# thowell/CALIPSO.jl

Hardware: AMD Instinct MI355X
Metric: Newton steps/sec (n~5k KKT) (higher is better)
Workload: dtype f64; 1 GPU; C3 synthetic dense conic QP: nx=2500 ne=1500 nc=1000 (400 R+ + 200 x SOC3), n=5000 condensed, N=8500 unreduced; ONE system per GPU stepped sequentially (replicas at N > 1); 1 LDL^T factorisation, 6 refinement round(s) per step; refinement_rounds=6

## Files before the change

calipso.jl_amd/csrc/api.hip:

```cpp
#include <algorithm>
#include <array>
#include <atomic>
#include <cmath>
#include <mutex>
#include <cstdio>
#include <cstdlib>
#include <cstring>

#include "internal.hpp"
#include "device_utils.hpp"
#include "host_logic.hpp"

using namespace calipso;

namespace calipso {
int check(H* s, hipError_t e, const char* what) {
    char buf[512];
    snprintf(buf, sizeof buf, "%s: %s", what, hipGetErrorString(e));
    if (s) s->err = buf;
    return CALIPSO_ERR_HIP;
}
bool lds_attribute(const void* kernel, int bytes) {
    static std::mutex mu;
    static std::map<std::pair<const void*, int>, std::pair<int, int>> done;
// ... 107 lines not shown
            const int st = d.ne + s->h_soc_start[j], dim = s->h_soc_dim[j];
            int lo = d.nx, hi = 0;
            for (int k = st; k < st + dim; ++k) if (zr[2 * (size_t)k + 1] > zr[2 * (size_t)k]) { lo = std::min(lo, zr[2 * (size_t)k]); hi = std::max(hi, zr[2 * (size_t)k + 1]); }
            for (int k = st; k < st + dim; ++k) { zr[2 * (size_t)k] = hi > lo ? lo : 0; zr[2 * (size_t)k + 1] = hi > lo ? hi : 0; }
        }
        if (spec->n_blocks < 1 || spec->block_start[0] != 1) { s->err = "calipso_hip_create_structured: hessian_block_start must begin with 1"; return CALIPSO_ERR_ARGUMENT; }
        for (int64_t b = 0; b < spec->n_blocks; ++b) {
            const int64_t c0 = spec->block_start[b], c1 = b + 1 < spec->n_blocks ? spec->block_start[b + 1] : nx + 1;
            if (c1 <= c0 || c1 > nx + 1) { s->err = "calipso_hip_create_structured: hessian_block_start must be increasing within 1..nx"; return CALIPSO_ERR_ARGUMENT; }
            for (int64_t c = c0; c < c1; ++c) lr[(size_t)c - 1] = (int)c1 - 2;
        }
        s->h_zrow = zr; s->h_lreach = lr;
        std::vector<int>& reach = s->h_reach;
        reach = lr;
        std::vector<int> ext((size_t)d.nx, -1);
        for (int k = 0; k < d.m; ++k) if (zr[2 * (size_t)k + 1] > zr[2 * (size_t)k]) ext[(size_t)zr[2 * (size_t)k]] = std::max(ext[(size_t)zr[2 * (size_t)k]], zr[2 * (size_t)k + 1] - 1);
        int run = -1;
        for (int j = 0; j < d.nx; ++j) { run = std::max(run, ext[(size_t)j]); if (run >= j) reach[(size_t)j] = std::max(reach[(size_t)j], run); }
        if (!calipso::blocks_plan(d, zr, lr, plan, s->err)) return CALIPSO_ERR_ARGUMENT;
        s->compact = true;
        s->blocks_zero_cell = plan.spacked - 1;
    }
    const bool cp = s->compact;
    std::vector<std::pair<double**, size_t>> carve;
    auto SL = [&](double** pp, size_t count) { carve.push_back({pp, count ? count : 1}); };
    double* icount_d = nullptr;
    SL(&s->Lxx, cp ? 1 : NX * NX); SL(&s->Lsym, cp ? plan.packed : NX * NX); SL(&s->Z, cp ? 1 : M * NX);
    SL(&s->fx, NX); SL(&s->gyx, NX); SL(&s->hzx, NX); SL(&s->gh, M);
    SL(&s->cone_product, NC); SL(&s->cone_target, NC); SL(&s->barrier_gradient, NC);
    SL(&s->dscal, 64); SL(&s->refpart, std::max((NE + NC + 255) / 256 + 1, M + 2) + (size_t)d.n_wide);
    SL(&s->solution, N); SL(&s->candidate, N); SL(&s->lambda, NE); SL(&s->parameters, (size_t)d.np);
    SL(&s->residual, N); SL(&s->residual_error, N); SL(&s->step, N); SL(&s->step_correction, N);
    SL(&s->saved_point, N); SL(&s->saved_g, NE); SL(&s->saved_h, NC);
    SL(&s->residual_symmetric, n); SL(&s->step_symmetric, n); SL(&s->merit_gradient, n);
    SL(&s->S, cp ? plan.spacked : NPd * NPd); SL(&s->Dx, NPd); SL(&s->Ypanel, cp ? 1 : NPd * NB);
    SL(&s->Tinv, cp ? 1 : calipso::tinv_doubles(d.NP)); SL(&s->Ttmp, cp ? 1 : NPd * 1024); SL(&s->zf2, NPd); SL(&s->WH, cp ? 1 : NC * NX);
    SL(&s->Wfac, (cp || !calipso::wform_layout_ok(d.NP, calipso::trsv_block(d.NP, 512))) ? 1 : NPd * NPd / 2);
    SL(&s->wz, NC); SL(&s->kzz, NC);
    SL(&s->Wsoc, (size_t)woff); SL(&s->Bsoc, (size_t)woff); SL(&s->socwork, (size_t)2 * woff);
    SL(&icount_d, 32);
    double* krange_d = nullptr;
    const size_t KG = (NX + 15) / 16;
    SL(&krange_d, 2 * KG);
    double* zrow_d = nullptr;
    SL(&zrow_d, M);
    const size_t maxdim = std::max(std::max(NX, M), NPd);
    SL(&s->gemv_partial, cp ? 1 : std::max(64 * maxdim, ((NX + 15) / 16) * M + ((M + 1023) / 1024) * NX));
    SL(&s->vtmp, 4 * std::max(N, NPd));
    SL(&s->xbuf, NPd); SL(&s->zf, NPd); SL(&s->t1, M); SL(&s->t2, M);
    SL(&s->zsx, M); SL(&s->w1, NX); SL(&s->w2, NX); SL(&s->lxv, NX);
    SL(&s->lgp, NX * d.np); SL(&s->gp, NE * d.np); SL(&s->hp, NC * d.np);
    SL(&s->jacobian_parameters, N * d.np); SL(&s->solution_sensitivity, N * d.np);
    SL(&s->qp.q, NX); SL(&s->qp.bh, M);
    size_t total = 0;
    for (auto& c : carve) total += (c.second + 31) & ~(size_t)31;
    CK(hipMalloc((void**)&s->slab, total * sizeof(double)));
    CK(hipMemsetAsync(s->slab, 0, total * sizeof(double), s->stream));
    s->slab_doubles = total;
    {
        size_t off = 0;
        for (auto& c : carve) { *c.first = s->slab + off; off += (c.second + 31) & ~(size_t)31; }
    }
    s->icount = reinterpret_cast<int*>(icount_d);
    s->krange = reinterpret_cast<int*>(krange_d);
    s->zrow = reinterpret_cast<int*>(zrow_d);
    s->gx = s->Z; s->hx = s->Z + NE; s->g = s->gh; s->hc = s->gh + NE;
    s->Lf = s->S;
    schur_plan(s);
    rc |= dalloc(s, &s->cone.soc_start, (size_t)d.n_soc); rc |= dalloc(s, &s->cone.soc_dim, (size_t)d.n_soc);
    rc |= dalloc(s, &s->cone.soc_woff, (size_t)d.n_soc); rc |= dalloc(s, &s->cone.entry_soc, NC);
    rc |= dalloc(s, &s->cone.wide, (size_t)d.n_wide);
    std::vector<int> zgrp;
    calipso::solve_tail_plan(d, s->h_soc_start, s->h_soc_dim, zgrp);
    if (zgrp.size() >= 2) { rc |= dalloc(s, &s->zgrp, zgrp.size()); s->n_zgrp = (int)zgrp.size() - 1; }
    rc |= dalloc(s, &s->gate, (size_t)4);
    if (rc) return CALIPSO_ERR_HIP;
    CK(hipHostMalloc((void**)&s->hscal, 64 * sizeof(double), hipHostMallocMapped | hipHostMallocCoherent));
    CK(hipHostMalloc((void**)&s->hicount, 64 * sizeof(int), hipHostMallocMapped | hipHostMallocCoherent));
    CK(hipHostMalloc((void**)&s->hseq, 64, hipHostMallocMapped | hipHostMallocCoherent));
    CK(hipHostGetDevicePointer((void**)&s->hscal_dev, s->hscal, 0));
    CK(hipHostGetDevicePointer((void**)&s->hicount_dev, s->hicount, 0));
    CK(hipHostGetDevicePointer((void**)&s->hseq_dev, s->hseq, 0));
    s->hseq[0] = 0;
    CK(hipStreamSynchronize(s->stream));
    {
        std::vector<int> kr(4 * KG);
        for (size_t g = 0; g < KG; ++g) { kr[4 * g] = 0; kr[4 * g + 1] = d.ne; kr[4 * g + 2] = 0; kr[4 * g + 3] = d.nc; }
        CK(hipMemcpy(s->krange, kr.data(), sizeof(int) * kr.size(), hipMemcpyHostToDevice));
    }
    if (s->zgrp) CK(hipMemcpy(s->zgrp, zgrp.data(), sizeof(int) * zgrp.size(), hipMemcpyHostToDevice));
    if (d.n_soc) {
        CK(hipMemcpy(s->cone.soc_start, s->h_soc_start.data(), sizeof(int) * d.n_soc, hipMemcpyHostToDevice));
        CK(hipMemcpy(s->cone.soc_dim, s->h_soc_dim.data(), sizeof(int) * d.n_soc, hipMemcpyHostToDevice));
        CK(hipMemcpy(s->cone.soc_woff, s->h_soc_woff.data(), sizeof(int) * d.n_soc, hipMemcpyHostToDevice));
    }
    if (d.n_wide) {
        std::vector<int> wide;
        for (int j = 0; j < d.n_soc; ++j) if (s->h_soc_dim[j] > 4) wide.push_back(j);
        CK(hipMemcpy(s->cone.wide, wide.data(), sizeof(int) * wide.size(), hipMemcpyHostToDevice));
    }
    std::vector<int> es((size_t)std::max(1, d.nc), -1);
    for (int j = 0; j < d.n_soc; ++j)
        for (int k = 0; k < s->h_soc_dim[j]; ++k) es[s->h_soc_start[j] + k] = j;
    if (d.nc) CK(hipMemcpy(s->cone.entry_soc, es.data(), sizeof(int) * d.nc, hipMemcpyHostToDevice));
    s->hpoint.assign(N, 0.0);
    s->hparams.assign((size_t)d.np, 0.0);
    Options& o = s->opt;
#define OD(f) s->optd["opt." #f] = &o.f
    OD(residual_norm); OD(constraint_norm); OD(scaling_line_search); OD(iterative_refinement_tolerance); OD(central_path_initial);
    OD(central_path_update_tolerance); OD(central_path_scaling); OD(central_path_exponent); OD(penalty_initial); OD(penalty_scaling);
    OD(dual_initial); OD(residual_tolerance); OD(optimality_tolerance); OD(slack_tolerance); OD(equality_tolerance);
    OD(complementarity_tolerance); OD(min_regularization); OD(primal_regularization_initial); OD(dual_regularization_initial);
    OD(max_regularization); OD(dual_regularization); OD(dual_regularization_exponent); OD(scaling_regularization_initial);
    OD(scaling_regularization); OD(scaling_regularization_last); OD(min_central_path); OD(max_penalty); OD(constraint_tensor);
    OD(update_factorization); OD(violation_tolerance); OD(violation_exponent); OD(merit_tolerance); OD(merit_exponent);
    OD(armijo_tolerance); OD(machine_tolerance); OD(max_filter); OD(differentiate); OD(warmstart);
#undef OD
    const int mf = (int)o.max_filter;
    s->filter_theta.assign(mf, 1.0e8); s->filter_merit.assign(mf, 1.0e8);
    s->cache_theta.assign(mf, 1.0e8); s->cache_merit.assign(mf, 1.0e8);
    if (cp) {
        CK(hipStreamSynchronize(s->stream));
        int brc = calipso::blocks_install(s, plan);
        if (brc < 0) return brc;
        brc = calipso_hip_set_stage_parallel(s, 1, 1, nullptr);
        if (brc < 0) return brc;
// ... 1210 lines not shown
```

calipso.jl_amd/csrc/gemv.hip:

```cpp
#include "internal.hpp"
#include "device_utils.hpp"

namespace calipso {

struct BlockRanges { int b0, b1, b2, b3; };
__device__ __forceinline__ BlockRanges column_blocks(const Sparsity& sp, int col, int rows) {
    BlockRanges r = {0, (rows + 63) / 64, 0, 0};
    if (sp.kind == SP_DENSE) return r;
    if (sp.kind == SP_LXX) { r.b0 = max(0, col - sp.hb) / 64; r.b1 = (min(rows, col + sp.hb + 1) + 63) / 64; return r; }
    const int* k = sp.kr + 4 * (col / 16);
    const int elo = k[0], ehi = k[1], clo = k[2], chi = k[3];
    if (sp.kind == SP_GX) { r.b0 = elo / 64; r.b1 = ehi > elo ? (ehi + 63) / 64 : r.b0; return r; }
    if (sp.kind == SP_HX) { r.b0 = clo / 64; r.b1 = chi > clo ? (chi + 63) / 64 : r.b0; return r; }
    r.b0 = elo / 64; r.b1 = ehi > elo ? (ehi + 63) / 64 : r.b0;
    r.b2 = (sp.ne + clo) / 64; r.b3 = chi > clo ? (sp.ne + chi + 63) / 64 : r.b2;
    return r;
}
__device__ __forceinline__ bool block_active(const BlockRanges& r, int b) { return (b >= r.b0 && b < r.b1) || (b >= r.b2 && b < r.b3); }

template <int NV>
__device__ __forceinline__ void structured_column(const BlockRanges& br, int rows, int lane, const double* __restrict__ a, const double* const (&x)[NV],
                                                  double (&acc0)[NV], double (&acc1)[NV]) {
#pragma unroll
    for (int pass = 0; pass < 2; ++pass) {
// ... 254 lines not shown
    for (int q = 0; q < BOTH_RQ; ++q) if (block_active(br, r0 / 64 + q)) active |= 1u << q;
    for (int j = c0; j < c1; ++j) {
        const double* a = A + (size_t)j * ld;
        double z[BOTH_RQ];
#pragma unroll
        for (int q = 0; q < BOTH_RQ; ++q) { const int i = r0 + lane + 64 * q; z[q] = (i < rows && ((active >> q) & 1u)) ? a[i] : 0.0; }
        const double xj = x[j];
        double t0 = 0.0, t1 = 0.0;
#pragma unroll
        for (int q = 0; q < BOTH_RQ; q += 2) {
            t0 += z[q] * uu[q]; t1 += z[q + 1] * uu[q + 1];
            acc[q] += z[q] * xj; acc[q + 1] += z[q + 1] * xj;
        }
        const double t = wave_sum(t0 + t1);
        if (lane == 0) part_t[(size_t)blockIdx.y * cols + j] = t;
    }
#pragma unroll
    for (int q = 0; q < BOTH_RQ; ++q) { const int i = r0 + lane + 64 * q; if (i < rows) part_n[(size_t)cg * rows + i] = acc[q]; }
}

void gemv_both(calipso_hip_solver* s, int rows, int cols, const double* A, int ld, const double* x, const double* u, double* yn, double* yt, double beta_t, int kind) {
    if (rows == 0 || cols == 0) return;
    if (s->compact) { s->err = "internal: a dense mat-vec was requested on a structured handle"; s->ldl_failed = true; return; }
    const BatchSc B = batch_of(s);
    const int cw = BOTH_CW;
    const int ncg = (cols + cw - 1) / cw, nrr = (rows + 64 * BOTH_RQ - 1) / (64 * BOTH_RQ);
    double* part_n = s->gemv_partial;
    double* part_t = s->gemv_partial + (size_t)ncg * rows;
    hipLaunchKernelGGL(k_gemv_both, dim3((ncg + 3) / 4, nrr, B.b.n), dim3(256), 0, s->stream, B.b, sparsity_of(s, kind), rows, cols, cw, A, ld, x, u, part_n, part_t);
    hipLaunchKernelGGL(k_gemv_n_reduce, dim3((rows + 63) / 64, 1, B.b.n), dim3(256), 0, s->stream, B.b, rows, ncg, part_n, yn, 1.0, 0.0);
    hipLaunchKernelGGL(k_gemv_n_reduce, dim3((cols + 63) / 64, 1, B.b.n), dim3(256), 0, s->stream, B.b, cols, nrr, part_t, yt, 1.0, beta_t);
}

static void gemv_n_chunks(int rows, int cols, int& rb, int& nchunk, int& chunk) {
    rb = (rows + GN_ROWS - 1) / GN_ROWS;
    nchunk = (768 + rb - 1) / rb;
    if (nchunk > GN_MAXCHUNK) nchunk = GN_MAXCHUNK;
    if (nchunk > (cols + 15) / 16) nchunk = (cols + 15) / 16;
    if (nchunk < 1) nchunk = 1;
    chunk = (cols + nchunk - 1) / nchunk;
    nchunk = (cols + chunk - 1) / chunk;
    if (cols == 0) nchunk = 0;
}

int gemv_refine_pair(calipso_hip_solver* s, const double* x1, const double* x2, double* y1, double* y2, const double* xl, double* yl, bool defer_reduce) {
    const Dims& d = s->d;
    if (d.m == 0 || s->blocks.on || s->compact) {
        if (d.m) gemv_t2(s, d.m, d.nx, s->Z, d.m, x1, x2, y1, y2, SP_Z);
        gemv_n(s, d.nx, d.nx, s->Lxx, d.nx, xl, yl, 1.0, 0.0, SP_LXX);
        return 0;
    }
    int rb, nchunk, chunk;
    gemv_n_chunks(d.nx, d.nx, rb, nchunk, chunk);
    const int nt2 = (d.nx + 3) / 4;
    const BatchSc B = batch_of(s);
    const bool timed = s->time_matvec && !s->cur;
    if (timed) (void)hipEventRecord(s->ev[5], s->stream);
    const size_t xbytes = 2 * sizeof(double) * (size_t)d.m;
    const int lds_x = gemv_lds_x(xbytes);
    hipLaunchKernelGGL(k_gemv_t2_and_n, dim3(nt2 + rb * nchunk, 1, B.b.n), dim3(256), lds_x ? xbytes : 0, s->stream, B.b, sparsity_of(s, SP_Z), d.m, d.nx, s->Z, d.m, x1, x2, y1, y2, nt2,
                       sparsity_of(s, SP_LXX), rb, d.nx, d.nx, chunk, s->Lxx, d.nx, xl, s->gemv_partial, s->gate_epoch ? s->gate : (const int*)nullptr, s->gate_epoch, lds_x);
    if (timed) { (void)hipEventRecord(s->ev[6], s->stream); s->time_matvec = false; s->matvec_timed = true; }
    if (defer_reduce) return nchunk;
    hipLaunchKernelGGL(k_gemv_n_reduce, dim3((d.nx + 63) / 64, 1, B.b.n), dim3(256), 0, s->stream, B.b, d.nx, nchunk, s->gemv_partial, yl, 1.0, 0.0);
    return 0;
}

void gemv_n(calipso_hip_solver* s, int rows, int cols, const double* A, int ld, const double* x, double* y, double alpha, double beta, int kind, const double* add) {
    if (rows == 0) return;
    if (blocks_gemv_n(s, kind, x, y, alpha, beta)) { if (add) launch_add(s, y, add, rows); return; }
    if (s->compact) { s->err = "internal: a dense mat-vec was requested on a structured handle"; s->ldl_failed = true; return; }
    int rb, nchunk, chunk;
    gemv_n_chunks(rows, cols, rb, nchunk, chunk);
    const BatchSc B = batch_of(s);
    if (nchunk > 0)
        hipLaunchKernelGGL(k_gemv_n_partial, dim3(rb, nchunk, B.b.n), dim3(GN_ROWS), 0, s->stream, B.b, sparsity_of(s, kind), kind == SP_HX ? s->d.ne : 0, rows, cols, chunk, A, ld,
                           x, s->gemv_partial);
    hipLaunchKernelGGL(k_gemv_n_reduce, dim3((rows + 63) / 64, 1, B.b.n), dim3(256), 0, s->stream, B.b, rows, nchunk, s->gemv_partial, y, alpha, beta, add);
}

}
```

calipso.jl_amd/csrc/internal.hpp:

```cpp
#pragma once
#include <hip/hip_runtime.h>
#include <stdint.h>

#include <map>
#include <string>
#include <vector>

#include "../../include/calipso_hip.h"
#include "../../include/calipso_options.hpp"

namespace calipso {

constexpr int TILE = 128;
constexpr int NB = 64;
constexpr int MAX_SOC_DIM = 1024;
constexpr int TRSV_BLOCK = 2048;
inline int trsv_block(int NP, int limit = TRSV_BLOCK) {
    if (NP <= 512) return NP;
    int tb = 512;
    while (2 * tb <= limit && 2 * tb <= NP) tb *= 2;
    for (;; tb /= 2) { const int rem = NP % tb; if (tb == 512 || (rem & (rem - 1)) == 0) return tb; }
}
inline size_t tinv_doubles(int NP) {
    size_t most = 0;
// ... 96 lines not shown
    calipso::Options opt;
    calipso::Scalars sc;
    calipso::ConeDev cone;
    calipso::QpEval qp;
    calipso::Stats stats;
    struct calipso_hip_group* owner = nullptr;
    const calipso::BatchSc* cur = nullptr;
    double* slab = nullptr; size_t slab_doubles = 0;
    int device = 0;
    hipStream_t stream = nullptr;
    std::string err;
    calipso_callback_fn cb_inner = nullptr, cb_outer = nullptr;
    void* cb_user = nullptr;
    calipso_device_eval_fn dev_eval = nullptr;
    void* dev_eval_user = nullptr;
    calipso_device_block_eval_fn dev_block_eval = nullptr;
    void* dev_block_eval_user = nullptr;
    size_t scratch_bytes = 0;
    bool rhs_ahead = false, rhs_joined = false;
    double *evalL = nullptr, *evalZ = nullptr;
    std::map<std::string, double*> optd;
    std::vector<int> h_soc_start, h_soc_dim, h_soc_woff;
    std::vector<int64_t> h_nonneg, h_soc_ptr, h_soc_idx;
    double* Lxx = nullptr;
    double* Z = nullptr;
    double *gx = nullptr, *hx = nullptr;
    double* Lsym = nullptr;
    bool hessian_dirty = true;
    double *fx = nullptr, *gyx = nullptr, *hzx = nullptr;
    double* gh = nullptr;
    double *g = nullptr, *hc = nullptr;
    double *cone_product = nullptr, *cone_target = nullptr, *barrier_gradient = nullptr;
    double* dscal = nullptr;
    double* hscal = nullptr;
    double* hscal_dev = nullptr;
    unsigned long long* hseq = nullptr;
    unsigned long long* hseq_dev = nullptr;
    unsigned long long pub_seq = 0;
    double *jacobian_parameters = nullptr, *solution_sensitivity = nullptr;
    double *solution = nullptr, *candidate = nullptr, *lambda = nullptr, *parameters = nullptr;
    double *residual = nullptr, *residual_error = nullptr, *step = nullptr, *step_correction = nullptr, *saved_point = nullptr;
    double *residual_symmetric = nullptr, *step_symmetric = nullptr, *merit_gradient = nullptr;
    bool pad_done = false;
    double* Kdense = nullptr;
    double* S = nullptr;
    double* Dx = nullptr;
    double* refpart = nullptr;
    int refparts = 0;
    int* zgrp = nullptr; int n_zgrp = 0;
    int* gate = nullptr; int gate_epoch = 0; int gate_counter = 0;
    bool refine_defer = false, refine_pending = false;
    bool spec_ahead_ok = false;
    bool refine_local_done = false;
    double* Ypanel = nullptr;
    double* Tinv = nullptr;
    double* Ttmp = nullptr;
    double* zf2 = nullptr;
    double* Wfac = nullptr;
    double* WH = nullptr;
    double* wz = nullptr;
    double* kzz = nullptr;
    double* Wsoc = nullptr;
    double* Bsoc = nullptr;
    double* socwork = nullptr;
    int schur_nj = 8;
    int half_bandwidth = 0, band64 = 0;
    std::vector<int> h_reach;
    std::vector<int> h_zrow, h_lreach;
    calipso::StageBlocks blocks;
    bool blocks_effective = true;
    size_t blocks_zero_cell = 0;
    bool compact = false;
    calipso_hip_sparse* spS = nullptr;
    long long* spS_src = nullptr;
    bool spS_values_current = false;
    int* spS_inv = nullptr;
    int* d_reach = nullptr;
    bool stage_parallel = false;
    calipso::i64 structure_resets = 0;
    int* krange = nullptr;
    int* zrow = nullptr;
    int* icount = nullptr;
    int* hicount = nullptr;
    int* hicount_dev = nullptr;
    double* gemv_partial = nullptr;
    double* vtmp = nullptr;
    double *xbuf = nullptr, *zf = nullptr, *t1 = nullptr, *t2 = nullptr;
    double *zsx = nullptr;
    double *w1 = nullptr, *w2 = nullptr, *lxv = nullptr;
    double *saved_g = nullptr, *saved_h = nullptr;
    double *lgp = nullptr, *gp = nullptr, *hp = nullptr;
    std::vector<double> hparams;
    double* multi_rhs = nullptr;
    double* dsym_multi = nullptr;
    void* scatter_aux = nullptr;
    void* ldl_aux = nullptr;
    void* lfac_aux = nullptr;
    bool lfac_last = false;
    bool lfac_failed = false;
    double* Lf = nullptr;
    double* Hdense = nullptr; int* lu_ipiv = nullptr;
    hipEvent_t ev[16];
    hipStream_t stream2 = nullptr;
    bool ldl_publish = false;
    unsigned long long ldl_pub_seq = 0;
    bool factor_times_pending = false;
// ... 158 lines not shown
```

calipso.jl_amd/csrc/vectors.hip:

```cpp
#include <algorithm>
#include <mutex>

#include "internal.hpp"
#include "device_utils.hpp"

namespace calipso {

constexpr int RT = 1024;

__global__ void k_residual(BatchSc bt, Dims d, const double* __restrict__ w, const double* __restrict__ lam,
                           const double* __restrict__ fx, const double* __restrict__ gyx, const double* __restrict__ hzx,
                           const double* __restrict__ g, const double* __restrict__ hc, const double* __restrict__ prod,
                           const double* __restrict__ targ, double* __restrict__ res) {
    inst_shift(bt.b, w, lam, fx, gyx, hzx, g, hc, prod, targ, res);
    const Scalars sc = bt.scal(blockIdx.z);
    const int i = blockIdx.x * blockDim.x + threadIdx.x;
    if (i >= d.N) return;
    double v;
    if (i < d.orr()) {
        v = fx[i];
        v += gyx[i];
        v += hzx[i];
    } else if (i < d.os()) {
        const int k = i - d.orr();
// ... 982 lines not shown
    double m = 0.0;
    double qs[MD], qt[MD], qz[MD];
#pragma unroll
    for (int a = 0; a < MD; ++a) { qs[a] = 0.0; qt[a] = 0.0; qz[a] = 0.0; }
#pragma unroll
    for (int a = 0; a < MD; ++a) if (a < dim) {
        const int k = st + a;
        const double hs = (0.0 + sc.ep) * lvs[a] - lvz[a] - lvt[a];
        qs[a] = res_s[a] - hs;
        const double hz = zk[a] + (-lvs[a] + (0.0 - sc.ed) * lvz[a]);
        qz[a] = res_z[a] - hz;
        double ht;
        if (a == 0) {
            ht = t[0] * lvs[0] + (sl[0] - sc.ed) * lvt[0];
#pragma unroll
            for (int q = 1; q < MD; ++q) if (q < dim) ht += t[q] * lvs[q] + sl[q] * lvt[q];
        } else {
            ht = t[a] * lvs[0] + sl[a] * lvt[0];
            ht += t[0] * lvs[a] + (sl[0] - sc.ed) * lvt[a];
        }
        qt[a] = res_t[a] - ht;
        A.e[d.os() + k] = qs[a]; A.e[d.oz() + k] = qz[a]; A.e[d.ot() + k] = qt[a];
        m = fmax(m, fmax(fmax(rabs(qs[a]), rabs(qz[a])), rabs(qt[a])));
    }
    double uu[MD], vv[MD], oo[MD];
#pragma unroll
    for (int a = 0; a < MD; ++a) { uu[a] = 0.0; vv[a] = 0.0; oo[a] = 0.0; }
    uu[0] = t[0] + sb1 * Hss;
#pragma unroll
    for (int k = 1; k < MD; ++k) if (k < dim) uu[k] = t[k] + sl[k] * Hss;
    double ac2 = sb1 * qs[0];
#pragma unroll
    for (int k = 1; k < MD; ++k) if (k < dim) ac2 += sl[k] * qs[k];
    vv[0] = ac2 + qt[0];
#pragma unroll
    for (int k = 1; k < MD; ++k) if (k < dim) vv[k] = (sl[k] * qs[0] + sb1 * qs[k]) + qt[k];
    arrow_inverse_small<MD>(dim, uu, vv, oo);
#pragma unroll
    for (int k = 0; k < MD; ++k) if (k < dim) { oo[k] = qz[k] + oo[k]; A.rsym[d.nx + d.ne + st + k] = oo[k]; }
#pragma unroll
    for (int a = 0; a < MD; ++a) if (a < dim) {
        double ss = 0.0;
#pragma unroll
        for (int b2 = 0; b2 < MD; ++b2) if (b2 < dim) ss += W[a + b2 * MD] * oo[b2];
        A.t1[d.ne + st + a] = ss;
    }
    return m;
}

#ifndef TAIL_EXP
#define TAIL_EXP 0
#endif
constexpr int TAIL_ROWS = 16, TAIL_PARTS = 32, TAIL_CPT = 16;
template <int PT>
__global__ __launch_bounds__(TAIL_ROWS * PT) void k_solve_tail(BatchSc bt, Dims d, ConeDev cd, const int* __restrict__ grp, int ngrp, const int* rowrange, const double* __restrict__ Z,
                                                                        const double* __restrict__ dx, const double* w, const double* res, const double* resid, const double* wz,
                                                                        const double* Wsoc, double* rsym, double* dsym, double* step, double* accum, double* zsx, double* e, double* t1,
                                                                        double* __restrict__ part, int zsx_mode, int do_refine, const int* __restrict__ gate = nullptr, int gate_epoch = 0) {
    if (gate && gate[0] == gate_epoch) return;
    constexpr int ROWS = TAIL_ROWS, PARTS = TAIL_PARTS, CPT = TAIL_CPT, W = PARTS * CPT, NS = PARTS / PT, HB = CPT / NS, NT = ROWS * PT;
    static_assert(PT == 32 || PT == 16, "one or two column parts per thread");
    extern __shared__ __attribute__((aligned(16))) double xs[];
    __shared__ double psum[PARTS][ROWS];
    __shared__ double t2s[ROWS];
    __shared__ double sm[ROWS * PARTS / 64];
    inst_shift(bt.b, Z, dx, w, res, resid, wz, Wsoc, rsym, dsym, step, zsx, e, t1, part);
    if (accum) inst_shift(bt.b, accum);
    if (rowrange) inst_shift_i(bt.b, rowrange);
    const Scalars sc = bt.scal(blockIdx.z);
    const int tid = threadIdx.x, r = tid % ROWS, p = tid / ROWS;
#if TAIL_EXP == 2
    const int per = (ngrp + 7) / 8, g = ((int)blockIdx.x & 7) * per + ((int)blockIdx.x >> 4), half = ((int)blockIdx.x >> 3) & 1;
#else
    const int per = (ngrp + 7) / 8, g = ((int)blockIdx.x & 7) * per + ((int)blockIdx.x >> 3);
#endif
    if (g >= ngrp) return;
    const int r0 = grp[g], nrows = grp[g + 1] - r0;
    const bool live = r < nrows;
    const double* Zr = Z + r0 + r;
    int jlo = 0, jhi = d.nx;
    if (rowrange && live) { jlo = rowrange[2 * (r0 + r)]; jhi = rowrange[2 * (r0 + r) + 1]; }
#if TAIL_EXP == 2
    { const int W2 = PARTS * CPT, np2 = (d.nx + W2 - 1) / W2, cut = ((np2 + 1) / 2) * W2; if (half == 0) jhi = cut; else jlo = cut; }
#endif
#if TAIL_EXP == 3
    jhi = 0;
#endif
    const int npass = (d.nx + W - 1) / W;
    const TailArgs A{w, res, resid, wz, Wsoc, rsym, dsym, step, accum, zsx, e, t1, zsx_mode, do_refine};
    TailPre P;
#if TAIL_EXP == 0
    if (tid < nrows) tail_prefetch(d, cd, A, r0 + tid, P);
#endif
    double va[NS][HB], vb[NS][HB];
    auto fetch = [&](int b, double (&v)[NS][HB]) {
        const int c0 = (b / NS) * W, q0 = (b % NS) * HB;
#pragma unroll
        for (int sl = 0; sl < NS; ++sl)
#pragma unroll
            for (int q = 0; q < HB; ++q) { const int c = c0 + (p + PT * sl) + PARTS * (q0 + q); v[sl][q] = (live && c < d.nx && c >= jlo && c < jhi) ? Zr[(size_t)c * d.m] : 0.0; }
    };
    const int nb = npass * NS;
    fetch(0, va);
    for (int i = tid; i < npass * W; i += NT) xs[i] = i < d.nx ? dx[i] : 0.0;
    __syncthreads();
    double acc[NS];
#pragma unroll
    for (int sl = 0; sl < NS; ++sl) acc[sl] = 0.0;
    auto sum = [&](int b, const double (&v)[NS][HB]) {
        const int c0 = (b / NS) * W, q0 = (b % NS) * HB;
#pragma unroll
        for (int sl = 0; sl < NS; ++sl)
#pragma unroll
            for (int q = 0; q < HB; ++q) acc[sl] += v[sl][q] * xs[c0 + (p + PT * sl) + PARTS * (q0 + q)];
    };
    for (int b = 0; b < nb; b += 2) {
        if (b + 1 < nb) fetch(b + 1, vb);
        sum(b, va);
        if (b + 1 < nb) {
            if (b + 2 < nb) fetch(b + 2, va);
            sum(b + 1, vb);
        }
    }
#pragma unroll
    for (int sl = 0; sl < NS; ++sl) psum[p + PT * sl][r] = acc[sl];
    {
        const int xsz = (d.nx + ngrp - 1) / ngrp, xend = min(d.nx, (g + 1) * xsz);
        for (int i = g * xsz + tid; i < xend; i += NT) {
            const double v = dx[i];
            dsym[i] = v; step[i] = v;
            if (accum) accum[i] += v;
        }
    }
    __syncthreads();
    if (tid < ROWS) {
        double s = 0.0;
#pragma unroll
        for (int q = 0; q < PARTS; ++q) s += psum[q][tid];
        t2s[tid] = s;
    }
    __syncthreads();
#if TAIL_EXP == 1 || TAIL_EXP == 2
    if (tid < nrows) t1[r0 + tid] = t2s[tid];
    return;
#endif
    double m = 0.0;
    if (tid < nrows) {
#if TAIL_EXP != 0
        tail_prefetch(d, cd, A, r0 + tid, P);
#endif
        const int row = r0 + tid;
        if (row < d.ne) m = tail_equality(d, sc, A, P, row, t2s[tid]);
        else if (row < d.ne + d.q) m = tail_nonnegative(d, sc, A, P, row - d.ne, t2s[tid]);
        else if (row - d.ne == P.st) m = tail_soc_small(d, sc, A, P, t2s + tid);
    }
    if (do_refine) {
        const double mr = block_max(m, sm);
        if (tid == 0) part[g] = mr;
    }
}
static bool solve_tail_ok(const calipso_hip_solver* s) {
    static const bool env = [] { const char* e = getenv("CALIPSO_HIP_SOLVE_TAIL"); return !e || atoi(e) != 0; }();
    return env && s->zgrp && s->d.m > 0 && !s->compact && !(s->blocks.on && s->blocks_effective);
}
bool solve_tail_available(const calipso_hip_solver* s) { return solve_tail_ok(s); }
bool launch_solve_tail(calipso_hip_solver* s, int which, bool accumulate, bool with_refine) {
    if (!solve_tail_ok(s)) return false;
    const BatchSc B = batch_of(s);
    const double* res = which == 0 ? s->residual : s->residual_error;
    double* st = which == 0 ? s->step : s->step_correction;
    constexpr int TW = TAIL_PARTS * TAIL_CPT;
    const size_t lds = sizeof(double) * (size_t)((s->d.nx + TW - 1) / TW) * TW;
    static const int env_pt = [] { const char* e = getenv("CALIPSO_HIP_TAIL_PT"); return e ? atoi(e) : 0; }();
    const bool narrow = env_pt ? env_pt == 16 : B.b.n >= 4;
    const void* fn = narrow ? (const void*)k_solve_tail<16> : (const void*)k_solve_tail<32>;
    if (lds > 48 * 1024) {
        if (lds > 96 * 1024 || !lds_attribute(fn, 96 * 1024)) return false;
    }
    const dim3 grid((s->n_zgrp + 7) / 8 * 8 * (TAIL_EXP == 2 ? 2 : 1), 1, B.b.n);
    auto go = [&](auto kern, int threads) {
        hipLaunchKernelGGL(kern, grid, dim3(threads), lds, s->stream, B, s->d, s->cone, s->zgrp, s->n_zgrp, s->band64 > 0 ? s->zrow : (const int*)nullptr, s->Z, s->xbuf, s->solution, res,
                           s->residual, s->wz, s->Wsoc, s->residual_symmetric, s->step_symmetric, st, accumulate ? s->step : (double*)nullptr, s->zsx, s->residual_error, s->t1, s->refpart,
                           which == 0 ? 1 : 2, with_refine ? 1 : 0, s->gate_epoch ? s->gate : (const int*)nullptr, s->gate_epoch);
    };
    if (narrow) go(k_solve_tail<16>, TAIL_ROWS * 16); else go(k_solve_tail<32>, TAIL_ROWS * 32);
    s->refine_local_done = with_refine;
    if (with_refine) s->refparts = s->n_zgrp;
    return true;
}
void solve_tail_plan(const Dims& d, const std::vector<int>& soc_start, const std::vector<int>& soc_dim, std::vector<int>& grp) {
    grp.clear();
    if (d.m == 0 || d.n_wide > 0) return;
    grp.push_back(0);
    int fill = 0, row = 0;
    auto item = [&](int size) {
        if (fill + size > TAIL_ROWS) { grp.push_back(row); fill = 0; }
        fill += size; row += size;
    };
    for (int k = 0; k < d.ne + d.q; ++k) item(1);
    for (size_t j = 0; j < soc_dim.size(); ++j) item(soc_dim[j]);
    grp.push_back(row);
    (void)soc_start;
}

void launch_refine_local(calipso_hip_solver* s) {
    if (s->refine_local_done) { s->refine_local_done = false; return; }
    const BatchSc B = batch_of(s);
    const int items = s->d.ne + s->d.q + s->d.n_soc;
    s->refparts = items ? (items + RL_THREADS - 1) / RL_THREADS + s->d.n_wide : 0;
    if (items == 0) return;
    hipLaunchKernelGGL(k_refine_local, dim3((items + RL_THREADS - 1) / RL_THREADS, 1, B.b.n), dim3(RL_THREADS), 0, s->stream, B, s->d, s->cone, s->solution, s->step,
                       s->residual, s->zsx, s->wz, s->Wsoc, s->residual_error, s->residual_symmetric, s->t1, s->refpart);
    launch_refine_local_wide(s, (items + RL_THREADS - 1) / RL_THREADS);
}
__global__ __launch_bounds__(256) void k_refine_x_fused(BatchSc bt, Dims d, int have_m, int nchunk, const double* __restrict__ partial, const double* __restrict__ v,
                                                         const double* __restrict__ res, const double* __restrict__ w1, const double* __restrict__ w2, double* __restrict__ e,
                                                         double* __restrict__ rsym, double* __restrict__ xbuf, double* __restrict__ dscal, const double* __restrict__ part, int nparts,
                                                         double* __restrict__ hpub, unsigned long long* __restrict__ hseq, unsigned long long seq, int* __restrict__ gate = nullptr,
                                                         int gate_epoch = 0, int it = -1, int min_it = 0, double tol = 0.0, int last_queued = 0) {
    __shared__ double ps[4][64];
    __shared__ double sm[4];
    __shared__ int last;
    inst_shift(bt.b, partial, v, res, w1, w2, e, rsym, xbuf, dscal, part);
    if (gate && gate[0] == gate_epoch) {
        if (last_queued && blockIdx.x == 0 && threadIdx.x == 0 && hpub) {
            hpub[7] = dscal[59]; hpub[20] = dscal[58]; hpub[21] = (double)gate[1]; hpub[22] = 1.0;
            __threadfence_system();
            __hip_atomic_store(hseq, seq, __ATOMIC_RELEASE, __HIP_MEMORY_SCOPE_SYSTEM);
        }
        return;
    }
    const Scalars sc = bt.scal(blockIdx.z);
    const int r = threadIdx.x & 63, p = threadIdx.x >> 6;
    const int i = blockIdx.x * 64 + r;
    double acc = 0.0;
    double w1i = 0.0, w2i = 0.0, vi0 = 0.0, resi = 0.0;
    if (p == 0 && i < d.nx) { w1i = have_m ? w1[i] : 0.0; w2i = have_m ? w2[i] : 0.0; vi0 = v[i]; resi = res[i]; }
    if (i < d.nx) {
        for (int c0 = p; c0 < nchunk; c0 += 64) {
            double pv[16];
#pragma unroll
            for (int u = 0; u < 16; ++u) { const int c = c0 + 4 * u; pv[u] = c < nchunk ? partial[(size_t)c * d.nx + i] : 0.0; }
#pragma unroll
            for (int u = 0; u < 16; ++u) if (c0 + 4 * u < nchunk) acc += pv[u];
        }
    }
    ps[p][r] = acc;
    __syncthreads();
    double m = 0.0;
    if (p == 0) {
        if (i < d.nx) {
            const double lv = (ps[0][r] + ps[1][r]) + (ps[2][r] + ps[3][r]);
            const double hv = (lv + w1i) + sc.ep * vi0;
            const double rr = resi - hv;
            e[i] = rr;
            rsym[i] = rr;
            xbuf[i] = have_m ? rr + w2i : rr;
            m = rabs(rr);
        } else if (i < d.NP) xbuf[i] = 0.0;
    }
    const double mr = block_max(m, sm);
    unsigned long long* nb = reinterpret_cast<unsigned long long*>(dscal + 60);
    unsigned* ticket = reinterpret_cast<unsigned*>(dscal + 61);
    if (threadIdx.x == 0) {
        atomicMax(nb, (unsigned long long)__double_as_longlong(mr));
        __threadfence();
        last = atomicAdd(ticket, 1u) == gridDim.x - 1;
    }
    __syncthreads();
    if (!last) return;
    double mm = 0.0;
    for (int k = threadIdx.x; k < nparts; k += 256) mm = fmax(mm, part[k]);
    const double mo = block_max(mm, sm);
    if (threadIdx.x == 0) {
        const double mx = fmax(mo, __longlong_as_double((long long)__hip_atomic_load(nb, __ATOMIC_RELAXED, __HIP_MEMORY_SCOPE_AGENT)));
        dscal[7] = mx;
        __hip_atomic_store(nb, 0ull, __ATOMIC_RELAXED, __HIP_MEMORY_SCOPE_AGENT);
        __hip_atomic_store(ticket, 0u, __ATOMIC_RELAXED, __HIP_MEMORY_SCOPE_AGENT);
        int stopped = 0;
        if (gate) {
            if (it == 0) dscal[58] = mx;
            dscal[59] = mx;
            gate[1] = it;
            if (mx <= tol && it >= min_it) { gate[0] = gate_epoch; stopped = 1; }
        }
        if (hpub && (!gate || last_queued)) {
            hpub[7] = mx;
            if (gate) { hpub[20] = dscal[58]; hpub[21] = (double)it; hpub[22] = (double)stopped; }
            __threadfence_system();
            __hip_atomic_store(hseq, seq, __ATOMIC_RELEASE, __HIP_MEMORY_SCOPE_SYSTEM);
        }
    }
}
void launch_refine_x_fused(calipso_hip_solver* s, bool publish, int nchunk, int it, bool last_queued) {
    const BatchSc B = batch_of(s);
    const bool spec = it >= 0 && s->gate_epoch != 0;
    const bool pub = publish && (!spec || last_queued);
    hipLaunchKernelGGL(k_refine_x_fused, dim3((s->d.NP + 63) / 64, 1, B.b.n), dim3(256), 0, s->stream, B, s->d, s->d.m > 0 ? 1 : 0, nchunk, s->gemv_partial, s->step, s->residual, s->w1, s->w2,
                       s->residual_error, s->residual_symmetric, s->xbuf, s->dscal, s->refpart, s->refparts, pub ? s->hscal_dev : (double*)nullptr,
                       pub ? s->hseq_dev : (unsigned long long*)nullptr, pub ? ++s->pub_seq : 0ULL, spec ? s->gate : (int*)nullptr, s->gate_epoch, it,
                       (int)s->opt.min_iterative_refinement, s->opt.iterative_refinement_tolerance, last_queued ? 1 : 0);
}
void launch_refine_x(calipso_hip_solver* s, bool publish) {
    const BatchSc B = batch_of(s);
    hipLaunchKernelGGL(k_refine_x, dim3(1, 1, B.b.n), dim3(RT), 0, s->stream, B, s->d, s->d.m > 0 ? 1 : 0, s->step, s->residual, s->lxv, s->w1, s->w2, s->residual_error,
                       s->residual_symmetric, s->xbuf, s->dscal, s->refpart, s->refparts,
                       publish ? s->hscal_dev : (double*)nullptr, publish ? s->hseq_dev : (unsigned long long*)nullptr, publish ? ++s->pub_seq : 0ULL);
}

__global__ void k_add(Batch bt, int n, double* __restrict__ y, const double* __restrict__ x) {
    inst_shift(bt, y, x);
    const int i = blockIdx.x * blockDim.x + threadIdx.x;
    if (i < n) y[i] += x[i];
}
void launch_add(calipso_hip_solver* s, double* y, const double* x, int len) {
    const BatchSc B = batch_of(s);
    hipLaunchKernelGGL(k_add, dim3((len + 255) / 256, 1, B.b.n), dim3(256), 0, s->stream, B.b, len, y, x);
}

__global__ void k_fill_d(Batch bt, double* __restrict__ p, size_t n, double v) {
    inst_shift(bt, p);
    const size_t i = (size_t)blockIdx.x * blockDim.x + threadIdx.x;
    if (i < n) p[i] = v;
}
__global__ void k_fill_i(Batch bt, int* __restrict__ p, size_t n, int v) {
    inst_shift_i(bt, p);
    const size_t i = (size_t)blockIdx.x * blockDim.x + threadIdx.x;
    if (i < n) p[i] = v;
}
__global__ void k_copy_d(Batch bt, double* __restrict__ dst, const double* __restrict__ src, size_t n) {
    inst_shift(bt, dst, src);
    const size_t i = (size_t)blockIdx.x * blockDim.x + threadIdx.x;
    if (i < n) dst[i] = src[i];
}
void fill_d(calipso_hip_solver* s, double* p, size_t n, double v) {
    if (!n) return;
    const BatchSc B = batch_of(s);
    hipLaunchKernelGGL(k_fill_d, dim3((unsigned)((n + 255) / 256), 1, B.b.n), dim3(256), 0, s->stream, B.b, p, n, v);
}
void fill_i(calipso_hip_solver* s, int* p, size_t n, int v) {
    if (!n) return;
    const BatchSc B = batch_of(s);
    hipLaunchKernelGGL(k_fill_i, dim3((unsigned)((n + 255) / 256), 1, B.b.n), dim3(256), 0, s->stream, B.b, p, n, v);
}
struct Copy4 { double* dst[4]; const double* src[4]; unsigned long long n[4]; };
__global__ void k_copy4_d(Batch bt, Copy4 c) {
    const int q = blockIdx.y;
    double* dst = c.dst[q]; const double* src = c.src[q];
    inst_shift(bt, dst, src);
    const size_t i = (size_t)blockIdx.x * blockDim.x + threadIdx.x;
    if (i < c.n[q]) dst[i] = src[i];
}
void copy4_d(calipso_hip_solver* s, double* const dst[4], const double* const src[4], const size_t n[4]) {
    Copy4 c; size_t nmax = 0;
// ... 47 lines not shown
```

Measured before the change: 545.8 Newton steps/s.

## Fold Z-transpose products into solve tail and keep Z slab resident in registers

The solve-tail kernel, which already streams rows of Z for the forward product, now also computes the two Z^T·v products per group. It uses DPP butterfly row sums and writes per-group partials, so the separate transposed GEMV pass in the refinement matvec is dropped (nt2=0). A register-resident slab variant keeps the Z tile loaded across both uses instead of fetching it twice, spilling it to LDS around the constraint code. k_refine_x_fused is templated to reduce these group partials in place of w1/w2. This removes a full extra read of Z per refinement round, at the cost of register pressure, extra partial-buffer traffic and a narrower reduce kernel.

```diff
diff --git a/calipso.jl_amd/csrc/api.hip b/calipso.jl_amd/csrc/api.hip
--- a/calipso.jl_amd/csrc/api.hip
+++ b/calipso.jl_amd/csrc/api.hip
@@ -183,6 +183,9 @@
     SL(&s->lgp, NX * d.np); SL(&s->gp, NE * d.np); SL(&s->hp, NC * d.np);
     SL(&s->jacobian_parameters, N * d.np); SL(&s->solution_sensitivity, N * d.np);
     SL(&s->qp.q, NX); SL(&s->qp.bh, M);
+    std::vector<int> zgrp;
+    calipso::solve_tail_plan(d, s->h_soc_start, s->h_soc_dim, zgrp);
+    SL(&s->ztpart, (cp || zgrp.size() < 2) ? 1 : 2 * (zgrp.size() - 1) * NX);
     size_t total = 0;
     for (auto& c : carve) total += (c.second + 31) & ~(size_t)31;
     CK(hipMalloc((void**)&s->slab, total * sizeof(double)));
@@ -201,8 +204,6 @@
     rc |= dalloc(s, &s->cone.soc_start, (size_t)d.n_soc); rc |= dalloc(s, &s->cone.soc_dim, (size_t)d.n_soc);
     rc |= dalloc(s, &s->cone.soc_woff, (size_t)d.n_soc); rc |= dalloc(s, &s->cone.entry_soc, NC);
     rc |= dalloc(s, &s->cone.wide, (size_t)d.n_wide);
-    std::vector<int> zgrp;
-    calipso::solve_tail_plan(d, s->h_soc_start, s->h_soc_dim, zgrp);
     if (zgrp.size() >= 2) { rc |= dalloc(s, &s->zgrp, zgrp.size()); s->n_zgrp = (int)zgrp.size() - 1; }
     rc |= dalloc(s, &s->gate, (size_t)4);
     if (rc) return CALIPSO_ERR_HIP;
diff --git a/calipso.jl_amd/csrc/gemv.hip b/calipso.jl_amd/csrc/gemv.hip
--- a/calipso.jl_amd/csrc/gemv.hip
+++ b/calipso.jl_amd/csrc/gemv.hip
@@ -330,12 +330,12 @@
     }
     int rb, nchunk, chunk;
     gemv_n_chunks(d.nx, d.nx, rb, nchunk, chunk);
-    const int nt2 = (d.nx + 3) / 4;
+    const int nt2 = s->zt_groups > 0 ? 0 : (d.nx + 3) / 4;
     const BatchSc B = batch_of(s);
     const bool timed = s->time_matvec && !s->cur;
     if (timed) (void)hipEventRecord(s->ev[5], s->stream);
     const size_t xbytes = 2 * sizeof(double) * (size_t)d.m;
-    const int lds_x = gemv_lds_x(xbytes);
+    const int lds_x = nt2 ? gemv_lds_x(xbytes) : 0;
     hipLaunchKernelGGL(k_gemv_t2_and_n, dim3(nt2 + rb * nchunk, 1, B.b.n), dim3(256), lds_x ? xbytes : 0, s->stream, B.b, sparsity_of(s, SP_Z), d.m, d.nx, s->Z, d.m, x1, x2, y1, y2, nt2,
                        sparsity_of(s, SP_LXX), rb, d.nx, d.nx, chunk, s->Lxx, d.nx, xl, s->gemv_partial, s->gate_epoch ? s->gate : (const int*)nullptr, s->gate_epoch, lds_x);
     if (timed) { (void)hipEventRecord(s->ev[6], s->stream); s->time_matvec = false; s->matvec_timed = true; }
diff --git a/calipso.jl_amd/csrc/internal.hpp b/calipso.jl_amd/csrc/internal.hpp
--- a/calipso.jl_amd/csrc/internal.hpp
+++ b/calipso.jl_amd/csrc/internal.hpp
@@ -172,6 +172,8 @@
     bool refine_defer = false, refine_pending = false;
     bool spec_ahead_ok = false;
     bool refine_local_done = false;
+    double* ztpart = nullptr;
+    int zt_groups = 0;
     double* Ypanel = nullptr;
     double* Tinv = nullptr;
     double* Ttmp = nullptr;
diff --git a/calipso.jl_amd/csrc/vectors.hip b/calipso.jl_amd/csrc/vectors.hip
--- a/calipso.jl_amd/csrc/vectors.hip
+++ b/calipso.jl_amd/csrc/vectors.hip
@@ -1058,20 +1058,50 @@
 #define TAIL_EXP 0
 #endif
 constexpr int TAIL_ROWS = 16, TAIL_PARTS = 32, TAIL_CPT = 16;
-template <int PT>
+template <int CTRL> __device__ __forceinline__ double zt_dpp(double v) {
+    const int lo = __double2loint(v), hi = __double2hiint(v);
+    return __hiloint2double(__builtin_amdgcn_update_dpp(hi, hi, CTRL, 0xf, 0xf, false), __builtin_amdgcn_update_dpp(lo, lo, CTRL, 0xf, 0xf, false));
+}
+__device__ __forceinline__ int zt_xor4_i(int v) {
+    const int t = __builtin_amdgcn_update_dpp(v, v, 0x104 , 0xf, 0x5, false);
+    return __builtin_amdgcn_update_dpp(t, v, 0x114 , 0xf, 0xa, false);
+}
+__device__ __forceinline__ double zt_xor4(double v) { return __hiloint2double(zt_xor4_i(__double2hiint(v)), zt_xor4_i(__double2loint(v))); }
+__device__ __forceinline__ int zt_slot(int r) { return (r & 3) | ((r & 8) >> 1) | ((r & 4) << 1); }
+__device__ __forceinline__ double zt_rowsum16(const double (&z)[16], double v, int r) {
+#pragma clang fp contract(off)
+    const bool b0 = r & 1, b1 = r & 2, b2 = r & 4, b3 = r & 8;
+    double a[8], b[4], c[2];
+#pragma unroll
+    for (int j = 0; j < 8; ++j) {
+        const double lo = z[2 * j] * v, hi = z[2 * j + 1] * v;
+        a[j] = (b0 ? hi : lo) + zt_dpp<0xB1 >(b0 ? lo : hi);
+    }
+#pragma unroll
+    for (int j = 0; j < 4; ++j) b[j] = (b1 ? a[2 * j + 1] : a[2 * j]) + zt_dpp<0x4E >(b1 ? a[2 * j] : a[2 * j + 1]);
+#pragma unroll
+    for (int j = 0; j < 2; ++j) c[j] = (b3 ? b[2 * j + 1] : b[2 * j]) + zt_dpp<0x128 >(b3 ? b[2 * j] : b[2 * j + 1]);
+    return (b2 ? c[1] : c[0]) + zt_xor4(b2 ? c[0] : c[1]);
+}
+constexpr int TAIL_SLAB_PASSES = 5;
+template <int PT, int RP = 0>
 __global__ __launch_bounds__(TAIL_ROWS * PT) void k_solve_tail(BatchSc bt, Dims d, ConeDev cd, const int* __restrict__ grp, int ngrp, const int* rowrange, const double* __restrict__ Z,
                                                                         const double* __restrict__ dx, const double* w, const double* res, const double* resid, const double* wz,
                                                                         const double* Wsoc, double* rsym, double* dsym, double* step, double* accum, double* zsx, double* e, double* t1,
-                                                                        double* __restrict__ part, int zsx_mode, int do_refine, const int* __restrict__ gate = nullptr, int gate_epoch = 0) {
+                                                                        double* __restrict__ part, int zsx_mode, int do_refine, double* __restrict__ ztpart = nullptr, const int* __restrict__ gate = nullptr,
+                                                                        int gate_epoch = 0) {
     if (gate && gate[0] == gate_epoch) return;
     constexpr int ROWS = TAIL_ROWS, PARTS = TAIL_PARTS, CPT = TAIL_CPT, W = PARTS * CPT, NS = PARTS / PT, HB = CPT / NS, NT = ROWS * PT;
     static_assert(PT == 32 || PT == 16, "one or two column parts per thread");
+    static_assert(RP == 0 || PT == 32, "the resident slab is the 512-thread form's");
+    static_assert(NS * HB == 16, "a batch is 16 columns per thread: one butterfly");
     extern __shared__ __attribute__((aligned(16))) double xs[];
     __shared__ double psum[PARTS][ROWS];
     __shared__ double t2s[ROWS];
     __shared__ double sm[ROWS * PARTS / 64];
     inst_shift(bt.b, Z, dx, w, res, resid, wz, Wsoc, rsym, dsym, step, zsx, e, t1, part);
     if (accum) inst_shift(bt.b, accum);
+    if (ztpart) inst_shift(bt.b, ztpart);
     if (rowrange) inst_shift_i(bt.b, rowrange);
     const Scalars sc = bt.scal(blockIdx.z);
     const int tid = threadIdx.x, r = tid % ROWS, p = tid / ROWS;
@@ -1107,7 +1137,17 @@
             for (int q = 0; q < HB; ++q) { const int c = c0 + (p + PT * sl) + PARTS * (q0 + q); v[sl][q] = (live && c < d.nx && c >= jlo && c < jhi) ? Zr[(size_t)c * d.m] : 0.0; }
     };
     const int nb = npass * NS;
-    fetch(0, va);
+    double slab[RP ? RP : 1][NS][HB];
+    if constexpr (RP > 0) {
+#pragma unroll
+        for (int b = 0; b < RP; ++b) {
+            if (b < nb) fetch(b, slab[b]);
+            else {
+#pragma unroll
+                for (int q = 0; q < HB; ++q) slab[b][0][q] = 0.0;
+            }
+        }
+    } else fetch(0, va);
     for (int i = tid; i < npass * W; i += NT) xs[i] = i < d.nx ? dx[i] : 0.0;
     __syncthreads();
     double acc[NS];
@@ -1120,6 +1160,10 @@
 #pragma unroll
             for (int q = 0; q < HB; ++q) acc[sl] += v[sl][q] * xs[c0 + (p + PT * sl) + PARTS * (q0 + q)];
     };
+    if constexpr (RP > 0) {
+#pragma unroll
+        for (int b = 0; b < RP; ++b) if (b < nb) sum(b, slab[b]);
+    } else
     for (int b = 0; b < nb; b += 2) {
         if (b + 1 < nb) fetch(b + 1, vb);
         sum(b, va);
@@ -1151,19 +1195,65 @@
     return;
 #endif
     double m = 0.0;
-    if (tid < nrows) {
+    auto constraints = [&] {
+        if (tid < nrows) {
 #if TAIL_EXP != 0
-        tail_prefetch(d, cd, A, r0 + tid, P);
+            tail_prefetch(d, cd, A, r0 + tid, P);
 #endif
-        const int row = r0 + tid;
-        if (row < d.ne) m = tail_equality(d, sc, A, P, row, t2s[tid]);
-        else if (row < d.ne + d.q) m = tail_nonnegative(d, sc, A, P, row - d.ne, t2s[tid]);
-        else if (row - d.ne == P.st) m = tail_soc_small(d, sc, A, P, t2s + tid);
-    }
+            const int row = r0 + tid;
+            if (row < d.ne) m = tail_equality(d, sc, A, P, row, t2s[tid]);
+            else if (row < d.ne + d.q) m = tail_nonnegative(d, sc, A, P, row - d.ne, t2s[tid]);
+            else if (row - d.ne == P.st) m = tail_soc_small(d, sc, A, P, t2s + tid);
+        }
+    };
+    if constexpr (RP > 0) {
+        if (tid < 64) {
+#pragma unroll
+            for (int b = 0; b < RP; ++b)
+#pragma unroll
+                for (int q = 0; q < HB; ++q) xs[(b * HB + q) * 64 + tid] = slab[b][0][q];
+            asm volatile("" ::: "memory");
+            constraints();
+            asm volatile("" ::: "memory");
+#pragma unroll
+            for (int b = 0; b < RP; ++b)
+#pragma unroll
+                for (int q = 0; q < HB; ++q) slab[b][0][q] = xs[(b * HB + q) * 64 + tid];
+        }
+    } else constraints();
     if (do_refine) {
         const double mr = block_max(m, sm);
         if (tid == 0) part[g] = mr;
     }
+    if (!(do_refine && ztpart)) return;
+    const double v1 = live ? (accum ? accum : step)[d.oy() + r0 + r] : 0.0, v2 = live ? t1[r0 + r] : 0.0;
+    double* zp1 = ztpart + (size_t)(2 * g) * d.nx;
+    double* zp2 = zp1 + d.nx;
+    const int slot = zt_slot(r);
+    auto apply = [&](int b, const double (&v)[NS][HB]) {
+        double z[16];
+#pragma unroll
+        for (int sl = 0; sl < NS; ++sl)
+#pragma unroll
+            for (int q = 0; q < HB; ++q) z[sl * HB + q] = v[sl][q];
+        const double s1 = zt_rowsum16(z, v1, r), s2 = zt_rowsum16(z, v2, r);
+        const int c = (b / NS) * W + (p + PT * (slot / HB)) + PARTS * ((b % NS) * HB + slot % HB);
+        if (c < d.nx) { zp1[c] = s1; zp2[c] = s2; }
+    };
+    if constexpr (RP > 0) {
+#pragma unroll
+        for (int b = 0; b < RP; ++b) if (b < nb) apply(b, slab[b]);
+    } else {
+        fetch(0, va);
+        for (int b = 0; b < nb; b += 2) {
+            if (b + 1 < nb) fetch(b + 1, vb);
+            apply(b, va);
+            if (b + 1 < nb) {
+                if (b + 2 < nb) fetch(b + 2, va);
+                apply(b + 1, vb);
+            }
+        }
+    }
 }
 static bool solve_tail_ok(const calipso_hip_solver* s) {
     static const bool env = [] { const char* e = getenv("CALIPSO_HIP_SOLVE_TAIL"); return !e || atoi(e) != 0; }();
@@ -1176,10 +1266,14 @@
     const double* res = which == 0 ? s->residual : s->residual_error;
     double* st = which == 0 ? s->step : s->step_correction;
     constexpr int TW = TAIL_PARTS * TAIL_CPT;
-    const size_t lds = sizeof(double) * (size_t)((s->d.nx + TW - 1) / TW) * TW;
+    size_t lds = sizeof(double) * (size_t)((s->d.nx + TW - 1) / TW) * TW;
     static const int env_pt = [] { const char* e = getenv("CALIPSO_HIP_TAIL_PT"); return e ? atoi(e) : 0; }();
     const bool narrow = env_pt ? env_pt == 16 : B.b.n >= 4;
-    const void* fn = narrow ? (const void*)k_solve_tail<16> : (const void*)k_solve_tail<32>;
+    static const bool env_slab = [] { const char* e = getenv("CALIPSO_HIP_TAIL_SLAB"); return !e || atoi(e) != 0; }();
+    const bool resident = !narrow && env_slab && s->d.nx <= TAIL_SLAB_PASSES * TW;
+    const bool zt = with_refine && s->ztpart && !s->blocks.on;
+    if (resident) lds = std::max(lds, sizeof(double) * 64 * TAIL_SLAB_PASSES * TAIL_CPT);
+    const void* fn = narrow ? (const void*)k_solve_tail<16> : resident ? (const void*)k_solve_tail<32, TAIL_SLAB_PASSES> : (const void*)k_solve_tail<32>;
     if (lds > 48 * 1024) {
         if (lds > 96 * 1024 || !lds_attribute(fn, 96 * 1024)) return false;
     }
@@ -1187,10 +1281,11 @@
     auto go = [&](auto kern, int threads) {
         hipLaunchKernelGGL(kern, grid, dim3(threads), lds, s->stream, B, s->d, s->cone, s->zgrp, s->n_zgrp, s->band64 > 0 ? s->zrow : (const int*)nullptr, s->Z, s->xbuf, s->solution, res,
                            s->residual, s->wz, s->Wsoc, s->residual_symmetric, s->step_symmetric, st, accumulate ? s->step : (double*)nullptr, s->zsx, s->residual_error, s->t1, s->refpart,
-                           which == 0 ? 1 : 2, with_refine ? 1 : 0, s->gate_epoch ? s->gate : (const int*)nullptr, s->gate_epoch);
+                           which == 0 ? 1 : 2, with_refine ? 1 : 0, zt ? s->ztpart : (double*)nullptr, s->gate_epoch ? s->gate : (const int*)nullptr, s->gate_epoch);
     };
-    if (narrow) go(k_solve_tail<16>, TAIL_ROWS * 16); else go(k_solve_tail<32>, TAIL_ROWS * 32);
+    if (narrow) go(k_solve_tail<16>, TAIL_ROWS * 16); else if (resident) go(k_solve_tail<32, TAIL_SLAB_PASSES>, TAIL_ROWS * 32); else go(k_solve_tail<32>, TAIL_ROWS * 32);
     s->refine_local_done = with_refine;
+    s->zt_groups = zt ? s->n_zgrp : 0;
     if (with_refine) s->refparts = s->n_zgrp;
     return true;
 }
@@ -1219,15 +1314,21 @@
                        s->residual, s->zsx, s->wz, s->Wsoc, s->residual_error, s->residual_symmetric, s->t1, s->refpart);
     launch_refine_local_wide(s, (items + RL_THREADS - 1) / RL_THREADS);
 }
+template <int RW, bool ZT>
 __global__ __launch_bounds__(256) void k_refine_x_fused(BatchSc bt, Dims d, int have_m, int nchunk, const double* __restrict__ partial, const double* __restrict__ v,
                                                          const double* __restrict__ res, const double* __restrict__ w1, const double* __restrict__ w2, double* __restrict__ e,
                                                          double* __restrict__ rsym, double* __restrict__ xbuf, double* __restrict__ dscal, const double* __restrict__ part, int nparts,
                                                          double* __restrict__ hpub, unsigned long long* __restrict__ hseq, unsigned long long seq, int* __restrict__ gate = nullptr,
-                                                         int gate_epoch = 0, int it = -1, int min_it = 0, double tol = 0.0, int last_queued = 0) {
-    __shared__ double ps[4][64];
+                                                         int gate_epoch = 0, int it = -1, int min_it = 0, double tol = 0.0, int last_queued = 0,
+                                                         const double* __restrict__ ztpart = nullptr, int ngrp = 0) {
+    constexpr int NL = 256 / RW;
+    static_assert(NL >= 4 && (!ZT || NL <= 16), "four lanes take the Hessian partials; a row's group sums fit one batch of loads");
+    __shared__ double ps[4][RW];
+    __shared__ double pz[ZT ? 2 * NL : 1][RW];
     __shared__ double sm[4];
     __shared__ int last;
     inst_shift(bt.b, partial, v, res, w1, w2, e, rsym, xbuf, dscal, part);
+    if (ZT) inst_shift(bt.b, ztpart);
     if (gate && gate[0] == gate_epoch) {
         if (last_queued && blockIdx.x == 0 && threadIdx.x == 0 && hpub) {
             hpub[7] = dscal[59]; hpub[20] = dscal[58]; hpub[21] = (double)gate[1]; hpub[22] = 1.0;
@@ -1237,12 +1338,25 @@
         return;
     }
     const Scalars sc = bt.scal(blockIdx.z);
-    const int r = threadIdx.x & 63, p = threadIdx.x >> 6;
-    const int i = blockIdx.x * 64 + r;
+    const int r = threadIdx.x % RW, p = threadIdx.x / RW;
+    const int i = blockIdx.x * RW + r;
     double acc = 0.0;
     double w1i = 0.0, w2i = 0.0, vi0 = 0.0, resi = 0.0;
-    if (p == 0 && i < d.nx) { w1i = have_m ? w1[i] : 0.0; w2i = have_m ? w2[i] : 0.0; vi0 = v[i]; resi = res[i]; }
-    if (i < d.nx) {
+    if (p == 0 && i < d.nx) { w1i = (have_m && !ZT) ? w1[i] : 0.0; w2i = (have_m && !ZT) ? w2[i] : 0.0; vi0 = v[i]; resi = res[i]; }
+    if constexpr (ZT) {
+        double a1 = 0.0, a2 = 0.0;
+        if (i < d.nx) {
+            for (int g0 = p; g0 < ngrp; g0 += 8 * NL) {
+                double u1[8], u2[8];
+#pragma unroll
+                for (int u = 0; u < 8; ++u) { const int g = g0 + NL * u; u1[u] = g < ngrp ? ztpart[(size_t)(2 * g) * d.nx + i] : 0.0; u2[u] = g < ngrp ? ztpart[(size_t)(2 * g + 1) * d.nx + i] : 0.0; }
+#pragma unroll
+                for (int u = 0; u < 8; ++u) if (g0 + NL * u < ngrp) { a1 += u1[u]; a2 += u2[u]; }
+            }
+        }
+        pz[p][r] = a1; pz[NL + p][r] = a2;
+    }
+    if (p < 4 && i < d.nx) {
         for (int c0 = p; c0 < nchunk; c0 += 64) {
             double pv[16];
 #pragma unroll
@@ -1251,11 +1365,15 @@
             for (int u = 0; u < 16; ++u) if (c0 + 4 * u < nchunk) acc += pv[u];
         }
     }
-    ps[p][r] = acc;
+    if (p < 4) ps[p][r] = acc;
     __syncthreads();
     double m = 0.0;
     if (p == 0) {
         if (i < d.nx) {
+            if constexpr (ZT) {
+#pragma unroll
+                for (int q = 0; q < NL; ++q) { w1i += pz[q][r]; w2i += pz[NL + q][r]; }
+            }
             const double lv = (ps[0][r] + ps[1][r]) + (ps[2][r] + ps[3][r]);
             const double hv = (lv + w1i) + sc.ep * vi0;
             const double rr = resi - hv;
@@ -1302,10 +1420,15 @@
     const BatchSc B = batch_of(s);
     const bool spec = it >= 0 && s->gate_epoch != 0;
     const bool pub = publish && (!spec || last_queued);
-    hipLaunchKernelGGL(k_refine_x_fused, dim3((s->d.NP + 63) / 64, 1, B.b.n), dim3(256), 0, s->stream, B, s->d, s->d.m > 0 ? 1 : 0, nchunk, s->gemv_partial, s->step, s->residual, s->w1, s->w2,
-                       s->residual_error, s->residual_symmetric, s->xbuf, s->dscal, s->refpart, s->refparts, pub ? s->hscal_dev : (double*)nullptr,
-                       pub ? s->hseq_dev : (unsigned long long*)nullptr, pub ? ++s->pub_seq : 0ULL, spec ? s->gate : (int*)nullptr, s->gate_epoch, it,
-                       (int)s->opt.min_iterative_refinement, s->opt.iterative_refinement_tolerance, last_queued ? 1 : 0);
+    const int ngrp = s->zt_groups;
+    s->zt_groups = 0;
+    auto go = [&](auto kern, int rw) {
+        hipLaunchKernelGGL(kern, dim3((s->d.NP + rw - 1) / rw, 1, B.b.n), dim3(256), 0, s->stream, B, s->d, s->d.m > 0 ? 1 : 0, nchunk, s->gemv_partial, s->step, s->residual, s->w1, s->w2,
+                           s->residual_error, s->residual_symmetric, s->xbuf, s->dscal, s->refpart, s->refparts, pub ? s->hscal_dev : (double*)nullptr,
+                           pub ? s->hseq_dev : (unsigned long long*)nullptr, pub ? ++s->pub_seq : 0ULL, spec ? s->gate : (int*)nullptr, s->gate_epoch, it,
+                           (int)s->opt.min_iterative_refinement, s->opt.iterative_refinement_tolerance, last_queued ? 1 : 0, s->ztpart, ngrp);
+    };
+    if (ngrp > 0) go(k_refine_x_fused<16, true>, 16); else go(k_refine_x_fused<64, false>, 64);
 }
 void launch_refine_x(calipso_hip_solver* s, bool publish) {
     const BatchSc B = batch_of(s);
```

Result: slower. 515.9 Newton steps/s (-5.5%).
